# TheaQG/DiffusionModelsCustom

Hardware: NVIDIA B200
Metric: samples_per_s_T1000_ddpm_sampling (higher is better)
Workload: dtype fp16 operands, fp32 accumulate (fp32 state/update)

## Files before the change

### diffusionmodelscustom_b200/_native.py

```python
from __future__ import annotations

import ctypes as C
import os

_PKG = os.path.dirname(os.path.abspath(__file__))
LIB_PATH = os.environ.get("B2D_LIB") or os.path.join(_PKG, "libb200ddpm.so")

FAMILY_R, FAMILY_D = 0, 1
INTERP_MODES = {"bicubic": 0, "bilinear": 1, "nearest": 2}

SYMBOLS = ["b2d_last_error", "b2d_abi_version", "b2d_create", "b2d_destroy", "b2d_load_weights", "b2d_set_schedule",
           "b2d_set_conditioning", "b2d_forward", "b2d_sample", "b2d_sample_host", "b2d_last_launch_count", "b2d_debug_read", "b2d_profile_step",
           "b2d_op_conv2d", "b2d_op_layernorm", "b2d_op_attention", "b2d_op_attn_block", "b2d_op_attn_block_out", "b2d_op_instnorm", "b2d_op_posterior_update", "b2d_saturation_count", "b2d_debug_attn_trace", "b2d_ensemble_run",
           "b2d_op_noise_image", "b2d_op_weighted_mse", "b2d_op_eval_daily", "b2d_op_eval_pixel", "b2d_op_histogram", "b2d_encoder_forward", "b2d_decoder_forward", "b2d_op_final_layer",
           "b2d_set_timesteps", "b2d_op_ddim_update"]


class Config(C.Structure):
    _fields_ = [(n, C.c_int32) for n in ("family", "img_size", "max_batch", "c_hr", "c_out", "has_lsm", "has_topo",
                                         "cond_channels", "num_classes", "n_heads", "attn_ff", "debug_simt_conv",
                                         "interp_mode", "stem_embedding")]


class Tensor(C.Structure):
    _fields_ = [("name", C.c_char_p), ("data", C.c_void_p), ("ndim", C.c_int32), ("shape", C.c_int64 * 4)]


class OpProfile(C.Structure):
    _fields_ = [("name", C.c_char * 48), ("klass", C.c_char * 24), ("flops", C.c_double), ("bytes", C.c_double),
                ("ms", C.c_double)]


class NativeError(RuntimeError):
    pass


_lib = None


def lib():
    global _lib
    if _lib is None:
        if not os.path.exists(LIB_PATH):
            raise NativeError(f"{LIB_PATH} is missing: build it with `python -m diffusionmodelscustom_b200.build` "
                              "(there is no fallback path)")
        L = C.CDLL(LIB_PATH)
# ... 8 lines not shown
                                           C.c_void_p, C.c_int32, C.c_void_p]
        L.b2d_forward.argtypes = [C.c_void_p, C.c_void_p, C.c_void_p, C.c_void_p, C.c_int32, C.c_void_p]
        L.b2d_sample.argtypes = [C.c_void_p, C.c_void_p, C.c_void_p, C.c_uint64, C.c_uint64, C.c_float, C.c_int32,
                                 C.c_void_p]
        L.b2d_sample_host.argtypes = [C.c_void_p, C.c_void_p, C.c_void_p, C.c_void_p, C.c_void_p, C.c_int32, C.c_int32,
                                      C.c_void_p, C.c_void_p, C.c_uint64, C.c_uint64, C.c_float, C.c_int32]
        L.b2d_last_launch_count.argtypes = [C.c_void_p]
        L.b2d_last_launch_count.restype = C.c_int64
        L.b2d_debug_read.argtypes = [C.c_void_p, C.c_char_p, C.c_void_p, C.c_int64, C.POINTER(C.c_int32), C.POINTER(C.c_int32)]
        L.b2d_profile_step.argtypes = [C.c_void_p, C.c_void_p, C.c_void_p, C.c_int32, C.c_int32, C.POINTER(OpProfile),
                                       C.c_int32, C.POINTER(C.c_int32)]
        L.b2d_op_conv2d.argtypes = [C.c_void_p] * 5 + [C.c_int32, C.c_void_p] + [C.c_int32] * 12 + [C.c_void_p]
        L.b2d_op_layernorm.argtypes = [C.c_void_p] * 4 + [C.c_int32, C.c_int32, C.c_void_p]
        L.b2d_op_attention.argtypes = [C.c_void_p, C.c_void_p] + [C.c_int32] * 4 + [C.c_void_p]
        L.b2d_op_attn_block.argtypes = [C.c_void_p] * 5 + [C.c_int32] * 4 + [C.c_void_p]
        L.b2d_op_attn_block_out.argtypes = [C.c_void_p] * 7 + [C.c_int32] * 5 + [C.c_void_p]
        L.b2d_op_instnorm.argtypes = [C.c_void_p, C.c_void_p, C.c_void_p, C.c_int32, C.c_void_p, C.c_void_p] + \
                                     [C.c_int32] * 3 + [C.c_void_p]
        L.b2d_op_final_layer.argtypes = [C.c_void_p] * 4 + [C.c_int32] * 4 + [C.c_void_p]
        L.b2d_op_posterior_update.argtypes = [C.c_void_p] * 6 + [C.c_int32, C.c_int32, C.c_int64, C.c_uint64, C.c_uint64,
                                                                 C.c_float, C.c_void_p]
        L.b2d_set_timesteps.argtypes = [C.c_void_p, C.c_void_p, C.c_int32, C.c_float]
        L.b2d_op_ddim_update.argtypes = [C.c_void_p] * 4 + [C.c_int32] * 3 + [C.c_float, C.c_int32, C.c_int64, C.c_uint64,
                                                              C.c_uint64, C.c_float, C.c_void_p]
        L.b2d_op_noise_image.argtypes = [C.c_void_p] * 6 + [C.c_int32, C.c_int64, C.c_uint64, C.c_uint64, C.c_float, C.c_void_p]
        L.b2d_op_weighted_mse.argtypes = [C.c_void_p] * 3 + [C.c_float, C.c_float, C.c_void_p, C.c_int64, C.c_void_p]
        L.b2d_op_eval_daily.argtypes = [C.c_void_p] * 4 + [C.c_int32, C.c_int64, C.c_void_p]
        L.b2d_op_eval_pixel.argtypes = [C.c_void_p] * 5 + [C.c_int32, C.c_int64, C.c_void_p]
        L.b2d_op_histogram.argtypes = [C.c_void_p, C.c_int64, C.c_float, C.c_float, C.c_int32, C.c_void_p, C.c_void_p]
        L.b2d_encoder_forward.argtypes = [C.c_void_p, C.c_void_p, C.c_void_p, C.POINTER(C.c_void_p), C.c_int32, C.c_void_p]
        L.b2d_decoder_forward.argtypes = [C.c_void_p, C.POINTER(C.c_void_p), C.c_void_p, C.c_void_p, C.c_int32, C.c_void_p]
        L.b2d_saturation_count.argtypes = [C.c_int32]
        L.b2d_saturation_count.restype = C.c_uint32
        if L.b2d_abi_version() != 1:
            raise NativeError("libb200ddpm.so ABI version mismatch")
        _lib = L
    return _lib


def check(rc: int):
    if rc != 0:
        raise NativeError(f"b200ddpm error {rc}: {lib().b2d_last_error().decode(errors='replace')}")


def ptr(t):
    return None if t is None else t.data_ptr()
```

### diffusionmodelscustom_b200/csrc/attention_tc8.cuh

```cuda
#pragma once
#include "attention_tc6.cuh"

namespace b2d {

constexpr int AT8_THREADS = 160;
constexpr int AT8_EQ_BYTES = ATC_BLK * ATC_D * 2;
constexpr int AT8_EK_BYTES = (ATC_BN / 2) * ATC_D * 2;
constexpr int AT8_SMEM = 1024 + ATC_TILE_BYTES + ATC_KV_BYTES * 3 * ATC_STAGES + AT8_EQ_BYTES + AT8_EK_BYTES + 256;

constexpr float AT8_OFF_SFU = 7.0f, AT8_OFF_POLY = 22.0f;

__device__ __forceinline__ uint32_t ex2_pair_poly_off(float xa, float xb) {
    uint32_t h, xr, nf, f, p, r;
    asm("cvt.rn.relu.f16x2.f32 %0, %1, %2;" : "=r"(h) : "f"(xb), "f"(xa));
    asm("add.rn.f16x2 %0, %1, %2;" : "=r"(xr) : "r"(h), "r"(0x66006600u));
    asm("sub.rn.f16x2 %0, %1, %2;" : "=r"(nf) : "r"(xr), "r"(0x66006600u));
    asm("sub.rn.f16x2 %0, %1, %2;" : "=r"(f) : "r"(h), "r"(nf));
    asm("fma.rn.f16x2 %0, %1, %2, %3;" : "=r"(p) : "r"(0x2B0D2B0Du), "r"(f), "r"(0x33C333C3u));
    asm("fma.rn.f16x2 %0, %1, %2, %3;" : "=r"(p) : "r"(p), "r"(f), "r"(0x398C398Cu));
    asm("fma.rn.f16x2 %0, %1, %2, %3;" : "=r"(p) : "r"(p), "r"(f), "r"(0x3C003C00u));
    const uint32_t e = xr * 1024u - 0x01980000u;
    asm("mul.rn.f16x2 %0, %1, %2;" : "=r"(r) : "r"(p), "r"(e));
    return r;
}

template <int POLY>
__global__ void __launch_bounds__(AT8_THREADS, AT6_CTAS_PER_SM)
    attn_tc8_kernel(const __grid_constant__ CUtensorMap tm, const __grid_constant__ CUtensorMap tmkv, f16* __restrict__ o, int L,
                    int C, float scale_log2e) {
    pdl_launch_dependents();
    extern __shared__ uint8_t at8_raw[];
    uint8_t* smem = reinterpret_cast<uint8_t*>((reinterpret_cast<uintptr_t>(at8_raw) + 1023) & ~uintptr_t(1023));
    uint8_t* sQ = smem;
    uint8_t* sK = sQ + ATC_TILE_BYTES;
    uint8_t* sV = sK + ATC_STAGES * ATC_KV_BYTES;
    uint8_t* sEq = sV + ATC_STAGES * 2 * ATC_KV_BYTES;
    uint8_t* sEk = sEq + AT8_EQ_BYTES;
    uint64_t* bars = reinterpret_cast<uint64_t*>(sEk + AT8_EK_BYTES);
    constexpr int KV_FULL = 0, S_FULL = 4 , P_EMPTY = 6, Q_FULL = 7, NBARS = 8;
    uint32_t* tmem_slot = reinterpret_cast<uint32_t*>(bars + NBARS);
    const uint32_t bar0 = smem_u32(bars);

    const int warp = threadIdx.x >> 5, lane = threadIdx.x & 31;
    const int head = blockIdx.y, b = blockIdx.z;
    const int q0 = blockIdx.x * ATC_BLK;
    const int nb = L / ATC_BN;
    const int row_base = b * L;
    constexpr int IW = 4, NT = AT8_THREADS;

    if (warp == IW) {
        if (lane == 0) {
            tma_prefetch_desc(&tm);
            tma_prefetch_desc(&tmkv);
            for (int i = 0; i < NBARS; ++i) mbar_init(&bars[i], 1);
            fence_mbar_init();
        }
        __syncwarp();
        tmem_alloc(tmem_slot, AT3_TMEM_COLS);
        tmem_relinquish();
    }
    for (int i = threadIdx.x; i < ATC_STAGES * ATC_BN * 2; i += NT) {
        const int st = i / (ATC_BN * 2), r = i % (ATC_BN * 2);
// ... 44 lines not shown
        }
        __syncwarp();
        named_bar_sync(4, NT);
        if (elect_one()) {
            issue_s_half(0, 0);
            issue_s_half(0, 1);
        }
        __syncwarp();
        for (int j = 0; j < nb; ++j) {
#pragma unroll
            for (int ch = 0; ch < 2; ++ch) {
                named_bar_sync(1 + ch, NT);
                tc_fence_after();
                if (j + 1 < nb) {
                    if (elect_one()) issue_s_half(j + 1, ch);
                    __syncwarp();
                }
            }
            named_bar_sync(3, NT);
            tc_fence_after();
            if (elect_one()) {
                const uint64_t dv = dv0 + (uint64_t)((j & (ATC_STAGES - 1)) * (2 * ATC_KV_BYTES / 16));
#pragma unroll
                for (int kk = 0; kk < ATC_BN / 16; ++kk)
                    umma_f16_ts(tmem + AT3_O_COL, tmem + AT3_P_COL + kk * 8, dv + (uint64_t)(kk * (512 / 16)), idesc_o, (j | kk) != 0);
                umma_commit_a(bar0 + 8 * P_EMPTY);
                if (j >= 1 && j + 3 < nb) load_kv(j + 3);
            }
            __syncwarp();
        }
    } else {
        const uint32_t tl = tmem + ((uint32_t)(warp * 32) << 16);
        const int row = warp * 32 + lane;
        {
            mbar_wait_a(bar0 + 8 * Q_FULL, 0);
            const f162 sc = __float2half2_rn(scale_log2e);
            f162* qp = reinterpret_cast<f162*>(sQ + threadIdx.x * 32);
#pragma unroll
            for (int i = 0; i < 8; ++i) qp[i] = __hmul2(qp[i], sc);
            fence_proxy_async();
            named_bar_arrive(4, NT);
        }
        uint32_t* eq_row = reinterpret_cast<uint32_t*>(sEq + row * 32);
        float m_ref = 0.f;
        float m_eq = 0.f;
        float mb[2] = {0.f, 0.f};
        auto rescale_o = [&](float fac) {
            uint32_t ov[32];
            tmem_ld32(tl + AT3_O_COL, ov);
            tmem_ld_wait();
            uint32_t o0[16], o1[16];
#pragma unroll
            for (int i = 0; i < 16; ++i) {
                o0[i] = __float_as_uint(__uint_as_float(ov[i]) * fac);
                o1[i] = __float_as_uint(__uint_as_float(ov[16 + i]) * fac);
            }
            tmem_st16(tl + AT3_O_COL, o0);
            tmem_st16(tl + AT3_O_COL + 16, o1);
            tmem_st_wait();
        };
        auto rescale_p_first_half = [&](float fac) {
            tmem_st_wait();
            uint32_t pv[32];
            tmem_ld32(tl + AT3_P_COL, pv);
            tmem_ld_wait();
            uint32_t p0[16];
#pragma unroll
            for (int i = 0; i < 16; ++i) {
                const float2 f = unpack_h2(pv[i]);
                p0[i] = pack_h2_nosat(f.x * fac, f.y * fac);
            }
            tmem_st16(tl + AT3_P_COL, p0);
        };

        for (int j = 0; j < nb; ++j) {
            bool waited_p = false;
#pragma unroll
            for (int ch = 0; ch < 2; ++ch) {
                mbar_wait_a(bar0 + 8 * (S_FULL + ch), j & 1);
                tc_fence_after();
                uint32_t v[32];
                tmem_ld32(tl + ch * 32, v);
                tmem_ld_wait();
                tc_fence_before();
                named_bar_arrive(1 + ch, NT);
                const float d0 = m_ref - mb[ch];
                mb[ch] = m_eq;
                float mx[2] = {-INFINITY, -INFINITY};
#pragma unroll
                for (int i = 0; i < 32; i += 2) {
                    const int cls = (((i >> 1) & 7) < POLY) ? 1 : 0;
                    mx[cls] = fmaxf(mx[cls], fmaxf(__uint_as_float(v[i]), __uint_as_float(v[i + 1])));
                }
                const bool first = (j == 0) && (ch == 0);
                const bool slow = d0 != 0.0f || mx[0] > 8.0f + AT8_OFF_SFU || mx[1] > 8.0f + AT8_OFF_POLY || first;
                if (__any_sync(0xffffffffu, slow)) {
                    const float cm = fmaxf(mx[0] - AT8_OFF_SFU, mx[1] - AT8_OFF_POLY) - d0;
                    const bool move = cm > 8.0f || first;
                    float m_new = m_ref;
                    if (move) {
                        const float t = m_ref + cm;
                        const f16 hi = __float2half_rn(t);
                        const f16 lo = __float2half_rn(t - __half2float(hi));
                        m_new = __half2float(hi) + __half2float(lo);
                    }
                    if (__any_sync(0xffffffffu, move)) {
                        if (!waited_p) {
                            mbar_wait_a(bar0 + 8 * P_EMPTY, (j & 1) ^ 1);
                            tc_fence_after();
                            waited_p = true;
                        }
                        const float fac = move ? ex2_approx(m_ref - m_new) : 1.0f;
                        if (j > 0) rescale_o(fac);
                        if (ch == 1) rescale_p_first_half(fac);
                        if (j + 1 < nb) mbar_wait_a(bar0 + 8 * (S_FULL + 0), (j + 1) & 1);
                        if (ch == 0) mbar_wait_a(bar0 + 8 * (S_FULL + 1), j & 1);
                        else if (j + 1 < nb) mbar_wait_a(bar0 + 8 * (S_FULL + 1), (j + 1) & 1);
                        if (move) {
                            const f16 hi = __float2half_rn(m_new);
                            const f16 lo = __float2half_rn(m_new - __half2float(hi));
                            const uint32_t w = (uint32_t)__half_as_ushort(__hneg(hi)) | ((uint32_t)__half_as_ushort(__hneg(lo)) << 16);
                            eq_row[0] = w;
                            eq_row[4] = w;
                            m_eq = m_new;
                        }
                        fence_proxy_async();
                    }
                    const float shift = m_new - (m_ref - d0);
#pragma unroll
                    for (int i = 0; i < 32; ++i) v[i] = __float_as_uint(__uint_as_float(v[i]) - shift);
                    m_ref = m_new;
                }
                uint32_t pk[16];
#pragma unroll
                for (int idx = 0; idx < 16 + AT_PIPE; ++idx) {
                    if (idx < 16) {
                        const float s0 = __uint_as_float(v[2 * idx]), s1 = __uint_as_float(v[2 * idx + 1]);
                        if ((idx & 7) < POLY) {
                            pk[idx] = ex2_pair_poly_off(s0, s1);
                        } else {
                            v[2 * idx] = __float_as_uint(ex2_ordered(s0));
                            v[2 * idx + 1] = __float_as_uint(ex2_ordered(s1));
                        }
                    }
                    if (idx >= AT_PIPE) {
                        const int i = idx - AT_PIPE;
                        if ((i & 7) >= POLY) pk[i] = pack_h2_ordered(__uint_as_float(v[2 * i]), __uint_as_float(v[2 * i + 1]));
                    }
                }
                if (!waited_p) {
                    mbar_wait_a(bar0 + 8 * P_EMPTY, (j & 1) ^ 1);
                    tc_fence_after();
                    waited_p = true;
                }
                tmem_st16(tl + AT3_P_COL + ch * 16, pk);
            }
            tmem_st_wait();
            tc_fence_before();
            named_bar_arrive(3, NT);
        }
        mbar_wait_a(bar0 + 8 * P_EMPTY, (nb - 1) & 1);
        tc_fence_after();
        uint32_t ov[32];
        tmem_ld32(tl + AT3_O_COL, ov);
        tmem_ld_wait();
        const float inv = 1.0f / __uint_as_float(ov[16]);
        f16* op = o + ((size_t)(row_base + q0 + row)) * C + head * ATC_D;
        uint4 o0, o1;
        o0.x = pack_h2(__uint_as_float(ov[0]) * inv, __uint_as_float(ov[1]) * inv);
        o0.y = pack_h2(__uint_as_float(ov[2]) * inv, __uint_as_float(ov[3]) * inv);
        o0.z = pack_h2(__uint_as_float(ov[4]) * inv, __uint_as_float(ov[5]) * inv);
        o0.w = pack_h2(__uint_as_float(ov[6]) * inv, __uint_as_float(ov[7]) * inv);
        o1.x = pack_h2(__uint_as_float(ov[8]) * inv, __uint_as_float(ov[9]) * inv);
        o1.y = pack_h2(__uint_as_float(ov[10]) * inv, __uint_as_float(ov[11]) * inv);
        o1.z = pack_h2(__uint_as_float(ov[12]) * inv, __uint_as_float(ov[13]) * inv);
        o1.w = pack_h2(__uint_as_float(ov[14]) * inv, __uint_as_float(ov[15]) * inv);
        reinterpret_cast<uint4*>(op)[0] = o0;
        reinterpret_cast<uint4*>(op)[1] = o1;
    }
    tc_fence_before();
    __syncthreads();
    if (warp == IW) {
        tc_fence_after();
        tmem_dealloc(tmem, AT3_TMEM_COLS);
    }
}

inline int attn_tc8_poly() {
    static const int v = [] {
        const char* e = getenv("B2D_ATTN_POLY");
        const int p = e ? atoi(e) : 4;
        return p < 0 ? 0 : (p > 5 ? 5 : p);
    }();
    return v;
}

template <int POLY>
inline int attn_tc8_attr() {
    B2D_CUDA(cudaFuncSetAttribute(attn_tc8_kernel<POLY>, cudaFuncAttributeMaxDynamicSharedMemorySize, AT8_SMEM));
    B2D_CUDA(cudaFuncSetAttribute(attn_tc8_kernel<POLY>, cudaFuncAttributePreferredSharedMemoryCarveout, cudaSharedmemCarveoutMaxShared));
    return 0;
}
inline int attn_tc8_init_attrs() {
    B2D_TRY(attn_tc8_attr<0>());
    B2D_TRY(attn_tc8_attr<2>());
    B2D_TRY(attn_tc8_attr<3>());
    B2D_TRY(attn_tc8_attr<4>());
    B2D_TRY(attn_tc8_attr<5>());
    return 0;
}

inline int attn_tc8_launch(const AttnTcMaps& m, f16* o, int B, int L, int C, int heads, cudaStream_t st) {
    const float scale_log2e = 1.4426950408889634f / sqrtf((float)ATC_D);
    const dim3 grid(L / ATC_BLK, heads, B), block(AT8_THREADS);
    switch (attn_tc8_poly()) {
        case 0: case 1: B2D_CUDA(launch_k(attn_tc8_kernel<0>, grid, block, AT8_SMEM, st, m.q, m.kv, o, L, C, scale_log2e)); break;
        case 2: B2D_CUDA(launch_k(attn_tc8_kernel<2>, grid, block, AT8_SMEM, st, m.q, m.kv, o, L, C, scale_log2e)); break;
        case 3: B2D_CUDA(launch_k(attn_tc8_kernel<3>, grid, block, AT8_SMEM, st, m.q, m.kv, o, L, C, scale_log2e)); break;
        case 4: B2D_CUDA(launch_k(attn_tc8_kernel<4>, grid, block, AT8_SMEM, st, m.q, m.kv, o, L, C, scale_log2e)); break;
        default: B2D_CUDA(launch_k(attn_tc8_kernel<5>, grid, block, AT8_SMEM, st, m.q, m.kv, o, L, C, scale_log2e)); break;
    }
    return 0;
}

}
```

### diffusionmodelscustom_b200/csrc/b200ddpm.cu

```cuda
#include "../../include/b200ddpm.h"

#include <chrono>
#include <cmath>
#include <cstring>
#include <functional>
#include <map>
#include <memory>
#include <vector>

#include "attention.cuh"
#include "attention_tc.cuh"
#include "attention_tc2.cuh"
#include "attention_tc3.cuh"
#include "attention_tc3d32.cuh"
#include "attention_tc6.cuh"
#include "attention_tc8.cuh"
#include "attn_block.cuh"
#include "common.cuh"
#include "conv.cuh"
#include "conv_persist.cuh"
#include "elementwise.cuh"
#include "evalops.cuh"
#include "gemm_stream.cuh"
#include "norm_fused.cuh"
// ... 488 lines not shown
            auto pl = std::make_shared<AttnBlockPlan>();
            if (attn_block_plan_build(*pl, x, W<f16>(role + ".qkvln.w"), W<float>(role + ".qkvln.c1"), W<float>(role + ".qkvln.b"), ao,
                                      rows, C, L, heads) != 0) { err = -1; return; }
            static const bool no_out_fuse = getenv("B2D_NO_ATTN_OUT_FUSE") != nullptr;
            static const int out_fuse_maxc = getenv("B2D_ATTN_OUT_FUSE_MAXC") ? atoi(getenv("B2D_ATTN_OUT_FUSE_MAXC")) : 128;
            static const bool want_gather = getenv("B2D_ATTN_GATHER") != nullptr;
            const bool gather = !no_out_fuse && want_gather && attn_block_gather_supported(C, heads);
            fused_out = gather || (!no_out_fuse && attn_block_out_supported(C, heads) && C <= out_fuse_maxc);
            double fl = 6.0 * rows * C * C + 4.0 * (double)L * L * C * B, by = 4.0 * rows * C + 6.0 * C * C;
            if (fused_out) {
                float* ws = nullptr;
                if (!gather && h->alloc(&ws, attn_block_ws_floats(rows, C, heads)) != 0) { err = -2; return; }
                if (attn_block_plan_fuse_out(*pl, W<f16>(role + ".out.w"), W<float>(role + ".out.b"), x,
                                             h->cfg.attn_ff ? s_mid : out, ws, h->cfg.attn_ff ? 0 : final_act, gather ? 2 : 1) != 0) { err = -1; return; }
                fl += 2.0 * rows * C * C;
                by += 4.0 * rows * C + 2.0 * C * C;
            }
            ops.meta(role + ".attn", "attn_block", fl, by);
            ops.push_back([=](cudaStream_t st) { return attn_block_launch(*pl, st); });
        } else if (fold) {
            next_ln_c1 = W<float>(role + ".qkvln.c1");
            conv(x, hw, hw, C, qkv, 3 * C, 1, 1, 0, false, role + ".qkvln", nullptr, nullptr, 0, 0);
        } else {
            ops.meta(role + ".ln", "layernorm", 0, 4.0 * rows * C);
            ops.push_back([=](cudaStream_t st) { return layernorm_launch(x, g, b, xn, rows, C, st); });
            conv(xn, hw, hw, C, qkv, 3 * C, 1, 1, 0, false, role + ".qkv", nullptr, nullptr, 0, 0);
        }
        static const bool no_tc_attn = getenv("B2D_NO_TC_ATTN") != nullptr;
        if (fused_block) {
        } else if (attn_tc_supported(L, C, heads) && !no_tc_attn) {
            auto tmq = std::make_shared<AttnTcMaps>();
            if (attn_tc_make_map(tmq.get(), qkv, B, L, C) != 0) { err = -1; return; }
            ops.meta(role + ".sdpa", "attn_tc", 4.0 * (double)L * L * C * B, 8.0 * rows * C);
            static const int attn_v = getenv("B2D_ATTN_V") ? atoi(getenv("B2D_ATTN_V")) : 8;
            const int sms = h->num_sms;
            if (attn_v == 2 && attn_tc2_supported(L, C, heads))
                ops.push_back([=](cudaStream_t st) { return attn_tc2_launch(*tmq, ao, Bc, L, C, heads, sms, st); });
            else if (attn_v == 1)
                ops.push_back([=](cudaStream_t st) { return attn_tc_launch(*tmq, ao, Bc, L, C, heads, st); });
            else if (attn_v == 4) {
                auto tm4 = std::make_shared<AttnTcMaps>();
                if (attn_tc4_make_map(tm4.get(), qkv, B, L, C) != 0) { err = -1; return; }
                ops.push_back([=](cudaStream_t st) { return attn_tc4_launch(*tm4, ao, Bc, L, C, heads, st); });
            } else if (attn_v == 6)
                ops.push_back([=](cudaStream_t st) { return attn_tc6_launch<0>(*tmq, ao, Bc, L, C, heads, st); });
            else if (attn_v == 7)
                ops.push_back([=](cudaStream_t st) { return attn_tc6_launch<1>(*tmq, ao, Bc, L, C, heads, st); });
            else if (attn_v == 8)
                ops.push_back([=](cudaStream_t st) { return attn_tc8_launch(*tmq, ao, Bc, L, C, heads, st); });
            else
                ops.push_back([=](cudaStream_t st) { return attn_tc3_launch(*tmq, ao, Bc, L, C, heads, st); });
        } else if (attn_tc5_supported(L, C, heads) && !no_tc_attn) {
            auto tm5 = std::make_shared<AttnTcMaps>();
            if (attn_tc5_make_map(tm5.get(), qkv, B, L, C) != 0) { err = -1; return; }
            ops.meta(role + ".sdpa", "attn_tc32", 4.0 * (double)L * L * C * B, 8.0 * rows * C);
            ops.push_back([=](cudaStream_t st) { return attn_tc5_launch(*tm5, ao, Bc, L, C, heads, st); });
        } else {
            ops.meta(role + ".sdpa", "flash_attn", 4.0 * (double)L * L * C * B, 8.0 * rows * C);
            ops.push_back([=](cudaStream_t st) { return flash_attn_launch(qkv, ao, Bc, L, C, heads, st); });
        }
        if (!h->cfg.attn_ff) {
            if (!fused_out) conv(ao, hw, hw, C, out, C, 1, 1, 0, false, role + ".out", x, nullptr, 0, final_act);
        } else {
            f16* mid = s_mid;
            f16* h1 = s_h1;
            if (!fused_out) conv(ao, hw, hw, C, mid, C, 1, 1, 0, false, role + ".out", x, nullptr, 0, 0);
            const float* g2 = W<float>(role + ".ffln.g");
            const float* b2 = W<float>(role + ".ffln.b");
            if (fold) {
                next_ln_c1 = W<float>(role + ".ff1ln.c1");
                conv(mid, hw, hw, C, h1, C, 1, 1, 0, false, role + ".ff1ln", nullptr, nullptr, 0, 2);
            } else {
                ops.meta(role + ".ffln", "layernorm", 0, 4.0 * rows * C);
                ops.push_back([=](cudaStream_t st) { return layernorm_launch(mid, g2, b2, xn, rows, C, st); });
                conv(xn, hw, hw, C, h1, C, 1, 1, 0, false, role + ".ff1", nullptr, nullptr, 0, 2);
            }
            conv(h1, hw, hw, C, out, C, 1, 1, 0, false, role + ".ff2", mid, nullptr, 0, final_act);
        }
    }

    float* stats_slice(int C) {
// ... 925 lines not shown
        return gemm_stream_launch(gp, as_stream(stream));
    }
    B2D_TRY(conv_tc_init_attrs());
    B2D_TRY(conv_plan_build(pl, sms, impl != 4 && impl != 5));
    if (impl == 5) impl = 3;
    if (impl == 3 || (impl == 0 && conv_tcp_eligible(pl, sms))) {
        B2D_CHECK(pl.p.splits == 1, "shape not eligible for the persistent convolution (split-K plan)");
        B2D_TRY(conv_tcp_init_attrs());
        return conv_launch_tcp(pl, sms, as_stream(stream));
    }
    float* ws = nullptr;
    if (pl.ws_floats) {
        B2D_CUDA(cudaMalloc(&ws, pl.ws_floats * sizeof(float)));
        pl.p.ws = ws;
    }
    int rc = conv_launch_tc(pl, as_stream(stream));
    if (ws) {
        cudaStreamSynchronize(as_stream(stream));
        cudaFree(ws);
    }
    return rc;
}

int b2d_op_layernorm(const void* x, const float* gamma, const float* beta, void* y, int32_t rows, int32_t C, void* stream) {
    return layernorm_launch((const f16*)x, gamma, beta, (f16*)y, rows, C, as_stream(stream));
}

int b2d_op_attention(const void* qkv, void* o, int32_t B, int32_t L, int32_t C, int32_t heads, void* stream) {
    B2D_TRY(flash_attn_init_attrs());
    if (attn_tc_supported(L, C, heads) && getenv("B2D_NO_TC_ATTN") == nullptr) {
        B2D_TRY(attn_tc_init_attrs());
        AttnTcMaps tm;
        B2D_TRY(attn_tc_make_map(&tm, (const f16*)qkv, B, L, C));
        const int attn_v = getenv("B2D_ATTN_V") ? atoi(getenv("B2D_ATTN_V")) : 8;
        if (attn_v == 3) {
            B2D_TRY(attn_tc3_init_attrs());
            return attn_tc3_launch(tm, (f16*)o, B, L, C, heads, as_stream(stream));
        }
        if (attn_v == 8) {
            B2D_TRY(attn_tc8_init_attrs());
            return attn_tc8_launch(tm, (f16*)o, B, L, C, heads, as_stream(stream));
        }
        if (attn_v == 6 || attn_v == 7) {
            B2D_TRY(attn_tc6_init_attrs());
            return attn_v == 6 ? attn_tc6_launch<0>(tm, (f16*)o, B, L, C, heads, as_stream(stream))
                               : attn_tc6_launch<1>(tm, (f16*)o, B, L, C, heads, as_stream(stream));
        }
        if (attn_v == 4) {
            B2D_TRY(attn_tc3_init_attrs());
            B2D_TRY(attn_tc4_make_map(&tm, (const f16*)qkv, B, L, C));
            return attn_tc4_launch(tm, (f16*)o, B, L, C, heads, as_stream(stream));
        }
        if (attn_v == 2 && attn_tc2_supported(L, C, heads)) {
            B2D_TRY(attn_tc2_init_attrs());
            int dev = 0, sms = 148;
            cudaGetDevice(&dev);
            cudaDeviceGetAttribute(&sms, cudaDevAttrMultiProcessorCount, dev);
            return attn_tc2_launch(tm, (f16*)o, B, L, C, heads, sms, as_stream(stream));
        }
        return attn_tc_launch(tm, (f16*)o, B, L, C, heads, as_stream(stream));
    }
    if (attn_tc5_supported(L, C, heads) && getenv("B2D_NO_TC_ATTN") == nullptr) {
        B2D_TRY(attn_tc5_init_attrs());
        AttnTcMaps tm5;
        B2D_TRY(attn_tc5_make_map(&tm5, (const f16*)qkv, B, L, C));
        return attn_tc5_launch(tm5, (f16*)o, B, L, C, heads, as_stream(stream));
    }
// ... 184 lines not shown
                      void* stream) {
    B2D_CHECK(gen && eval && mae_out && rmse_out && n_samples >= 1 && hw >= 1, "bad argument");
    eval_daily_kernel<<<n_samples, 256, 0, as_stream(stream)>>>(gen, eval, mae_out, rmse_out, (size_t)hw);
    B2D_CUDA(cudaGetLastError());
    return 0;
}

int b2d_op_eval_pixel(const float* gen, const float* eval, float* mae_out, float* rmse_out, float* bias_out, int32_t n_samples,
                      int64_t hw, void* stream) {
    B2D_CHECK(gen && eval && mae_out && rmse_out && bias_out && n_samples >= 1 && hw >= 1, "bad argument");
    eval_pixel_kernel<<<(unsigned)((hw + 255) / 256), 256, 0, as_stream(stream)>>>(gen, eval, mae_out, rmse_out, bias_out, n_samples, (size_t)hw);
    B2D_CUDA(cudaGetLastError());
    return 0;
}

int b2d_op_histogram(const float* x, int64_t n, float lo, float hi, int32_t bins, unsigned long long* counts_dev, void* stream) {
    B2D_CHECK(x && counts_dev && n >= 0 && bins >= 1 && bins <= HIST_MAX_BINS && hi > lo, "bad argument");
    cudaStream_t st = as_stream(stream);
    B2D_CUDA(cudaMemsetAsync(counts_dev, 0, (size_t)bins * 8, st));
    if (n == 0) return 0;
    const int blocks = (int)std::min<int64_t>((n + 255) / 256, 148 * 4);
    histogram_kernel<<<blocks, 256, (size_t)bins * 4, st>>>(x, (size_t)n, lo, hi, bins, counts_dev);
    B2D_CUDA(cudaGetLastError());
    return 0;
}

int b2d_debug_attn_trace(long long* out_host, int32_t max_elems) {
    B2D_CHECK(out_host && max_elems >= AT2_TRACE_BLOCKS * 12, "trace buffer too small");
    B2D_CUDA(cudaDeviceSynchronize());
    B2D_CUDA(cudaMemcpyFromSymbol(out_host, g_at2_trace, sizeof(long long) * AT2_TRACE_BLOCKS * 12));
    return AT2_TRACE_BLOCKS;
}

unsigned int b2d_saturation_count(int32_t reset) {
    unsigned int v = 0;
    if (cudaMemcpyFromSymbol(&v, g_sat_count, sizeof(v)) != cudaSuccess) return 0xFFFFFFFFu;
    if (reset) {
        const unsigned int z = 0;
        cudaMemcpyToSymbol(g_sat_count, &z, sizeof(z));
    }
    return v;
}

}
```

### include/b200ddpm.h

```cpp
#ifndef B200DDPM_H
#define B200DDPM_H

#include <stddef.h>
#include <stdint.h>

#ifdef __cplusplus
extern "C" {
#endif

#define B2D_ABI_VERSION 1

typedef struct b2d_handle b2d_handle;

enum { B2D_FAMILY_R = 0,
       B2D_FAMILY_D = 1   };

typedef struct b2d_config {
    int32_t family;
    int32_t img_size;
    int32_t max_batch;
    int32_t c_hr;
    int32_t c_out;
    int32_t has_lsm;
    int32_t has_topo;
// ... 38 lines not shown
int b2d_set_timesteps(b2d_handle* h, const int32_t* timesteps_host, int32_t n, float eta);
int b2d_op_ddim_update(float* x, const float* eps, const float* z_or_null, const float* alpha_hat, int32_t T, int32_t t,
                       int32_t t_prev, float eta, int32_t B, int64_t per_sample, uint64_t seed, uint64_t sample_offset,
                       float noise_scale, void* stream);

int b2d_sample_host(b2d_handle* h, float* x_inout_host, const float* lsm_host, const float* topo_host,
                    const float* cond_host, int32_t cond_h, int32_t cond_w, const int64_t* y_host,
                    const float* noise_host, uint64_t seed, uint64_t sample_offset, float noise_scale, int32_t B);

typedef struct b2d_ensemble_job {
    int32_t n_dates, members, sub_batch;
    int32_t first, count;
    const float* lsm;
    const float* topo;
    const float* cond;
    int32_t cond_h, cond_w;
    const int64_t* y;
    float* out;
    uint64_t seed;
    float noise_scale;
    float xT_scale;
} b2d_ensemble_job;
typedef struct b2d_ensemble_stats {
    int32_t sub_batches;
    int32_t out_pinned;
    int64_t launches;
    double gather_ms;
    double wall_ms;
} b2d_ensemble_stats;
int b2d_ensemble_run(b2d_handle* h, const b2d_ensemble_job* job, b2d_ensemble_stats* stats);

unsigned int b2d_saturation_count(int32_t reset);

int64_t b2d_last_launch_count(const b2d_handle* h);
typedef struct b2d_op_profile {
    char name[48];
    char klass[24];
    double flops;
    double bytes;
    double ms;
} b2d_op_profile;
int b2d_profile_step(b2d_handle* h, const float* x, const int64_t* t_host, int32_t B, int32_t reps, b2d_op_profile* out,
                     int32_t max_ops, int32_t* n_ops);

int b2d_debug_read(b2d_handle* h, const char* name, float* out_host, int64_t max_elems, int32_t* C_out, int32_t* hw_out);

int b2d_op_noise_image(const float* x0, const int64_t* t_dev, const float* alpha_hat, const float* noise_or_null, float* x_t,
                       float* noise_out, int32_t B, int64_t per_sample, uint64_t seed, uint64_t sample_offset, float noise_scale,
                       void* stream);
int b2d_op_weighted_mse(const float* input, const float* target, const float* sdf_or_null, float max_land_weight,
                        float min_sea_weight, float* out_scalar_dev, int64_t n, void* stream);
int b2d_op_eval_daily(const float* gen, const float* eval, float* mae_out, float* rmse_out, int32_t n_samples, int64_t hw,
                      void* stream);
int b2d_op_eval_pixel(const float* gen, const float* eval, float* mae_out, float* rmse_out, float* bias_out, int32_t n_samples,
                      int64_t hw, void* stream);
int b2d_op_histogram(const float* x, int64_t n, float lo, float hi, int32_t bins, unsigned long long* counts_dev, void* stream);

int b2d_debug_attn_trace(long long* out_host, int32_t max_elems);

int b2d_op_conv2d(const void* in_f16, const void* w_packed_f16, const float* bias, const void* residual_f16,
                  const float* post_add, int32_t post_stride, void* out_f16, int32_t B, int32_t Hi, int32_t Wi,
                  int32_t Cin, int32_t Cout, int32_t R, int32_t S, int32_t stride, int32_t pad, int32_t convt,
                  int32_t act, int32_t impl, void* stream);
int b2d_op_layernorm(const void* x_f16, const float* gamma, const float* beta, void* y_f16, int32_t rows, int32_t C,
                     void* stream);
int b2d_op_attention(const void* qkv_f16, void* o_f16, int32_t B, int32_t L, int32_t C, int32_t heads, void* stream);
// ... 18 lines not shown
```

Before: 25.82.

## Skip per-tile softmax max scan using Cauchy-Schwarz bound from key-norm table

Adds a pre-pass kernel that computes, for every 32-key tile and head, an upper bound on the key norms. The attention kernel computes each query's norm and uses the product as a bound on the scores, so the per-chunk row-max reduction and rescale logic run only when that bound could exceed the current reference. This removes max-scan work from the softmax warps, at the cost of an extra launch, an allocation and a table read per chunk. It is enabled by default (variant 9) only when L is at least 4096, and optional atomic counters can record how often the slow path runs.

After: 26.43, median of 6. 1.02x the previous value.

```diff
diff --git a/diffusionmodelscustom_b200/_native.py b/diffusionmodelscustom_b200/_native.py
--- a/diffusionmodelscustom_b200/_native.py
+++ b/diffusionmodelscustom_b200/_native.py
@@ -11,7 +11,7 @@
 
 SYMBOLS = ["b2d_last_error", "b2d_abi_version", "b2d_create", "b2d_destroy", "b2d_load_weights", "b2d_set_schedule",
            "b2d_set_conditioning", "b2d_forward", "b2d_sample", "b2d_sample_host", "b2d_last_launch_count", "b2d_debug_read", "b2d_profile_step",
-           "b2d_op_conv2d", "b2d_op_layernorm", "b2d_op_attention", "b2d_op_attn_block", "b2d_op_attn_block_out", "b2d_op_instnorm", "b2d_op_posterior_update", "b2d_saturation_count", "b2d_debug_attn_trace", "b2d_ensemble_run",
+           "b2d_op_conv2d", "b2d_op_layernorm", "b2d_op_attention", "b2d_op_attn_block", "b2d_op_attn_block_out", "b2d_op_instnorm", "b2d_op_posterior_update", "b2d_saturation_count", "b2d_op_attn_kmax", "b2d_attn_scan_stats", "b2d_debug_attn_trace", "b2d_ensemble_run",
            "b2d_op_noise_image", "b2d_op_weighted_mse", "b2d_op_eval_daily", "b2d_op_eval_pixel", "b2d_op_histogram", "b2d_encoder_forward", "b2d_decoder_forward", "b2d_op_final_layer",
            "b2d_set_timesteps", "b2d_op_ddim_update"]
 
@@ -86,6 +86,8 @@
         L.b2d_decoder_forward.argtypes = [C.c_void_p, C.POINTER(C.c_void_p), C.c_void_p, C.c_void_p, C.c_int32, C.c_void_p]
         L.b2d_saturation_count.argtypes = [C.c_int32]
         L.b2d_saturation_count.restype = C.c_uint32
+        L.b2d_op_attn_kmax.argtypes = [C.c_void_p, C.c_void_p] + [C.c_int32] * 3 + [C.c_void_p]
+        L.b2d_attn_scan_stats.argtypes = [C.c_int32, C.POINTER(C.c_uint64)]
         if L.b2d_abi_version() != 1:
             raise NativeError("libb200ddpm.so ABI version mismatch")
         _lib = L
diff --git a/diffusionmodelscustom_b200/csrc/attention_tc8.cuh b/diffusionmodelscustom_b200/csrc/attention_tc8.cuh
--- a/diffusionmodelscustom_b200/csrc/attention_tc8.cuh
+++ b/diffusionmodelscustom_b200/csrc/attention_tc8.cuh
@@ -24,10 +24,14 @@
     return r;
 }
 
-template <int POLY>
+__device__ unsigned long long g_attn_scan[4];
+
+__device__ __forceinline__ float at8_bound_limit(float m_ref) { return m_ref + 8.0f - 0x1p-8f - fabsf(m_ref) * 0x1p-10f; }
+
+template <int POLY, bool BOUND>
 __global__ void __launch_bounds__(AT8_THREADS, AT6_CTAS_PER_SM)
     attn_tc8_kernel(const __grid_constant__ CUtensorMap tm, const __grid_constant__ CUtensorMap tmkv, f16* __restrict__ o, int L,
-                    int C, float scale_log2e) {
+                    int C, float scale_log2e, const float* __restrict__ kmax, unsigned long long* __restrict__ stats) {
     pdl_launch_dependents();
     extern __shared__ uint8_t at8_raw[];
     uint8_t* smem = reinterpret_cast<uint8_t*>((reinterpret_cast<uintptr_t>(at8_raw) + 1023) & ~uintptr_t(1023));
@@ -138,12 +142,22 @@
     } else {
         const uint32_t tl = tmem + ((uint32_t)(warp * 32) << 16);
         const int row = warp * 32 + lane;
+        float qn_up = 0.f;
         {
             mbar_wait_a(bar0 + 8 * Q_FULL, 0);
             const f162 sc = __float2half2_rn(scale_log2e);
             f162* qp = reinterpret_cast<f162*>(sQ + threadIdx.x * 32);
-#pragma unroll
-            for (int i = 0; i < 8; ++i) qp[i] = __hmul2(qp[i], sc);
+            float qq = 0.f;
+#pragma unroll
+            for (int i = 0; i < 8; ++i) {
+                const f162 sq = __hmul2(qp[i], sc);
+                qp[i] = sq;
+                if constexpr (BOUND) {
+                    const float2 f = __half22float2(sq);
+                    qq = fmaf(f.x, f.x, fmaf(f.y, f.y, qq));
+                }
+            }
+            qn_up = sqrtf(qq) * (1.0f + 0x1p-10f);
             fence_proxy_async();
             named_bar_arrive(4, NT);
         }
@@ -151,6 +165,8 @@
         float m_ref = 0.f;
         float m_eq = 0.f;
         float mb[2] = {0.f, 0.f};
+        float lim = at8_bound_limit(m_ref);
+        const float* kt = kmax + ((size_t)b * gridDim.y + head) * (L / 32);
         auto rescale_o = [&](float fac) {
             uint32_t ov[32];
             tmem_ld32(tl + AT3_O_COL, ov);
@@ -183,6 +199,8 @@
             bool waited_p = false;
 #pragma unroll
             for (int ch = 0; ch < 2; ++ch) {
+                float km = 0.f;
+                if constexpr (BOUND) km = __ldg(kt + 2 * j + ch);
                 mbar_wait_a(bar0 + 8 * (S_FULL + ch), j & 1);
                 tc_fence_after();
                 uint32_t v[32];
@@ -192,50 +210,68 @@
                 named_bar_arrive(1 + ch, NT);
                 const float d0 = m_ref - mb[ch];
                 mb[ch] = m_eq;
-                float mx[2] = {-INFINITY, -INFINITY};
-#pragma unroll
-                for (int i = 0; i < 32; i += 2) {
-                    const int cls = (((i >> 1) & 7) < POLY) ? 1 : 0;
-                    mx[cls] = fmaxf(mx[cls], fmaxf(__uint_as_float(v[i]), __uint_as_float(v[i + 1])));
-                }
                 const bool first = (j == 0) && (ch == 0);
-                const bool slow = d0 != 0.0f || mx[0] > 8.0f + AT8_OFF_SFU || mx[1] > 8.0f + AT8_OFF_POLY || first;
-                if (__any_sync(0xffffffffu, slow)) {
-                    const float cm = fmaxf(mx[0] - AT8_OFF_SFU, mx[1] - AT8_OFF_POLY) - d0;
-                    const bool move = cm > 8.0f || first;
-                    float m_new = m_ref;
-                    if (move) {
-                        const float t = m_ref + cm;
-                        const f16 hi = __float2half_rn(t);
-                        const f16 lo = __float2half_rn(t - __half2float(hi));
-                        m_new = __half2float(hi) + __half2float(lo);
+                bool over = false, need = true;
+                if constexpr (BOUND) {
+                    over = !(qn_up * km <= lim);
+                    need = first || d0 != 0.0f || over;
+                }
+                if (!BOUND || __any_sync(0xffffffffu, need)) {
+                    if (BOUND && stats != nullptr) {
+                        const unsigned ob = __ballot_sync(0xffffffffu, over);
+                        if (lane == 0) {
+                            atomicAdd(&stats[1], 1ull);
+                            if (ob) {
+                                atomicAdd(&stats[2], 1ull);
+                                atomicAdd(&stats[3], (unsigned long long)__popc(ob));
+                            }
+                        }
                     }
-                    if (__any_sync(0xffffffffu, move)) {
-                        if (!waited_p) {
-                            mbar_wait_a(bar0 + 8 * P_EMPTY, (j & 1) ^ 1);
-                            tc_fence_after();
-                            waited_p = true;
+                    float mx[2] = {-INFINITY, -INFINITY};
+#pragma unroll
+                    for (int i = 0; i < 32; i += 2) {
+                        const int cls = (((i >> 1) & 7) < POLY) ? 1 : 0;
+                        mx[cls] = fmaxf(mx[cls], fmaxf(__uint_as_float(v[i]), __uint_as_float(v[i + 1])));
+                    }
+                    const bool slow = d0 != 0.0f || mx[0] > 8.0f + AT8_OFF_SFU || mx[1] > 8.0f + AT8_OFF_POLY || first;
+                    if (__any_sync(0xffffffffu, slow)) {
+                        const float cm = fmaxf(mx[0] - AT8_OFF_SFU, mx[1] - AT8_OFF_POLY) - d0;
+                        const bool move = cm > 8.0f || first;
+                        float m_new = m_ref;
+                        if (move) {
+                            const float t = m_ref + cm;
+                            const f16 hi = __float2half_rn(t);
+                            const f16 lo = __float2half_rn(t - __half2float(hi));
+                            m_new = __half2float(hi) + __half2float(lo);
                         }
-                        const float fac = move ? ex2_approx(m_ref - m_new) : 1.0f;
-                        if (j > 0) rescale_o(fac);
-                        if (ch == 1) rescale_p_first_half(fac);
-                        if (j + 1 < nb) mbar_wait_a(bar0 + 8 * (S_FULL + 0), (j + 1) & 1);
-                        if (ch == 0) mbar_wait_a(bar0 + 8 * (S_FULL + 1), j & 1);
-                        else if (j + 1 < nb) mbar_wait_a(bar0 + 8 * (S_FULL + 1), (j + 1) & 1);
-                        if (move) {
-                            const f16 hi = __float2half_rn(m_new);
-                            const f16 lo = __float2half_rn(m_new - __half2float(hi));
-                            const uint32_t w = (uint32_t)__half_as_ushort(__hneg(hi)) | ((uint32_t)__half_as_ushort(__hneg(lo)) << 16);
-                            eq_row[0] = w;
-                            eq_row[4] = w;
-                            m_eq = m_new;
+                        if (__any_sync(0xffffffffu, move)) {
+                            if (!waited_p) {
+                                mbar_wait_a(bar0 + 8 * P_EMPTY, (j & 1) ^ 1);
+                                tc_fence_after();
+                                waited_p = true;
+                            }
+                            const float fac = move ? ex2_approx(m_ref - m_new) : 1.0f;
+                            if (j > 0) rescale_o(fac);
+                            if (ch == 1) rescale_p_first_half(fac);
+                            if (j + 1 < nb) mbar_wait_a(bar0 + 8 * (S_FULL + 0), (j + 1) & 1);
+                            if (ch == 0) mbar_wait_a(bar0 + 8 * (S_FULL + 1), j & 1);
+                            else if (j + 1 < nb) mbar_wait_a(bar0 + 8 * (S_FULL + 1), (j + 1) & 1);
+                            if (move) {
+                                const f16 hi = __float2half_rn(m_new);
+                                const f16 lo = __float2half_rn(m_new - __half2float(hi));
+                                const uint32_t w = (uint32_t)__half_as_ushort(__hneg(hi)) | ((uint32_t)__half_as_ushort(__hneg(lo)) << 16);
+                                eq_row[0] = w;
+                                eq_row[4] = w;
+                                m_eq = m_new;
+                            }
+                            fence_proxy_async();
                         }
-                        fence_proxy_async();
+                        const float shift = m_new - (m_ref - d0);
+#pragma unroll
+                        for (int i = 0; i < 32; ++i) v[i] = __float_as_uint(__uint_as_float(v[i]) - shift);
+                        m_ref = m_new;
+                        if constexpr (BOUND) lim = at8_bound_limit(m_ref);
                     }
-                    const float shift = m_new - (m_ref - d0);
-#pragma unroll
-                    for (int i = 0; i < 32; ++i) v[i] = __float_as_uint(__uint_as_float(v[i]) - shift);
-                    m_ref = m_new;
                 }
                 uint32_t pk[16];
 #pragma unroll
@@ -283,6 +319,7 @@
         o1.w = pack_h2(__uint_as_float(ov[14]) * inv, __uint_as_float(ov[15]) * inv);
         reinterpret_cast<uint4*>(op)[0] = o0;
         reinterpret_cast<uint4*>(op)[1] = o1;
+        if (BOUND && stats != nullptr && lane == 0) atomicAdd(&stats[0], 2ull * nb);
     }
     tc_fence_before();
     __syncthreads();
@@ -301,32 +338,92 @@
     return v;
 }
 
-template <int POLY>
+__global__ void __launch_bounds__(1024) attn_kmax_kernel(const f16* __restrict__ qkv, float* __restrict__ kmax, int L, int C) {
+    pdl_launch_dependents();
+    __shared__ unsigned s_max[32];
+    const int heads = C / ATC_D, h0 = blockIdx.y * 32;
+    const int hn = heads - h0 < 32 ? heads - h0 : 32;
+    const int r = threadIdx.x / hn, hd = threadIdx.x - r * hn;
+    const size_t key = (size_t)blockIdx.x * 32 + r;
+    if (threadIdx.x < hn) s_max[threadIdx.x] = 0u;
+    pdl_wait();
+    const uint4* kp = reinterpret_cast<const uint4*>(qkv + key * 3 * C + C + (h0 + hd) * ATC_D);
+    const uint4 a = __ldg(kp), c = __ldg(kp + 1);
+    const uint32_t w[8] = {a.x, a.y, a.z, a.w, c.x, c.y, c.z, c.w};
+    float s = 0.f;
+#pragma unroll
+    for (int i = 0; i < 8; ++i) {
+        const float2 f = unpack_h2(w[i]);
+        s = fmaf(f.x, f.x, fmaf(f.y, f.y, s));
+    }
+    float n = sqrtf(s) * (1.0f + 0x1p-10f);
+    if (!(n <= INFINITY)) n = INFINITY;
+    __syncthreads();
+    atomicMax(&s_max[hd], __float_as_uint(n));
+    __syncthreads();
+    if (threadIdx.x < hn) {
+        const int b = (int)((size_t)blockIdx.x * 32 / L), t = (int)((size_t)blockIdx.x % (L / 32));
+        kmax[((size_t)b * heads + h0 + threadIdx.x) * (L / 32) + t] = __uint_as_float(s_max[threadIdx.x]);
+    }
+}
+
+inline bool attn_tc8_bound_pays(int L) { return L >= 4096; }
+
+inline size_t attn_kmax_floats(int B, int L, int C) { return (size_t)B * (C / ATC_D) * (L / 32); }
+
+inline int attn_kmax_launch(const f16* qkv, float* kmax, int B, int L, int C, cudaStream_t st) {
+    B2D_CHECK(C > 0 && C % ATC_D == 0 && L > 0 && L % 32 == 0, "shape not eligible for the key-norm table");
+    const int heads = C / ATC_D;
+    B2D_CUDA(launch_k(attn_kmax_kernel, dim3(B * (L / 32), (heads + 31) / 32), dim3(32 * (heads < 32 ? heads : 32)), 0, st, qkv, kmax, L, C));
+    return 0;
+}
+
+inline bool& attn_scan_stats_on() {
+    static bool on = false;
+    return on;
+}
+inline unsigned long long* attn_scan_stats_ptr() {
+    if (!attn_scan_stats_on()) return nullptr;
+    void* p = nullptr;
+    return cudaGetSymbolAddress(&p, g_attn_scan) == cudaSuccess ? static_cast<unsigned long long*>(p) : nullptr;
+}
+
+template <int POLY, bool BOUND>
 inline int attn_tc8_attr() {
-    B2D_CUDA(cudaFuncSetAttribute(attn_tc8_kernel<POLY>, cudaFuncAttributeMaxDynamicSharedMemorySize, AT8_SMEM));
-    B2D_CUDA(cudaFuncSetAttribute(attn_tc8_kernel<POLY>, cudaFuncAttributePreferredSharedMemoryCarveout, cudaSharedmemCarveoutMaxShared));
+    B2D_CUDA(cudaFuncSetAttribute(attn_tc8_kernel<POLY, BOUND>, cudaFuncAttributeMaxDynamicSharedMemorySize, AT8_SMEM));
+    B2D_CUDA(cudaFuncSetAttribute(attn_tc8_kernel<POLY, BOUND>, cudaFuncAttributePreferredSharedMemoryCarveout, cudaSharedmemCarveoutMaxShared));
     return 0;
 }
+template <bool BOUND>
+inline int attn_tc8_attrs() {
+    B2D_TRY((attn_tc8_attr<0, BOUND>()));
+    B2D_TRY((attn_tc8_attr<2, BOUND>()));
+    B2D_TRY((attn_tc8_attr<3, BOUND>()));
+    B2D_TRY((attn_tc8_attr<4, BOUND>()));
+    B2D_TRY((attn_tc8_attr<5, BOUND>()));
+    return 0;
+}
 inline int attn_tc8_init_attrs() {
-    B2D_TRY(attn_tc8_attr<0>());
-    B2D_TRY(attn_tc8_attr<2>());
-    B2D_TRY(attn_tc8_attr<3>());
-    B2D_TRY(attn_tc8_attr<4>());
-    B2D_TRY(attn_tc8_attr<5>());
-    return 0;
-}
-
-inline int attn_tc8_launch(const AttnTcMaps& m, f16* o, int B, int L, int C, int heads, cudaStream_t st) {
+    B2D_TRY(attn_tc8_attrs<false>());
+    return attn_tc8_attrs<true>();
+}
+
+template <bool BOUND>
+inline int attn_tc8_launch_t(const AttnTcMaps& m, f16* o, int B, int L, int C, int heads, const float* kmax, cudaStream_t st) {
     const float scale_log2e = 1.4426950408889634f / sqrtf((float)ATC_D);
     const dim3 grid(L / ATC_BLK, heads, B), block(AT8_THREADS);
+    unsigned long long* stats = BOUND ? attn_scan_stats_ptr() : nullptr;
     switch (attn_tc8_poly()) {
-        case 0: case 1: B2D_CUDA(launch_k(attn_tc8_kernel<0>, grid, block, AT8_SMEM, st, m.q, m.kv, o, L, C, scale_log2e)); break;
-        case 2: B2D_CUDA(launch_k(attn_tc8_kernel<2>, grid, block, AT8_SMEM, st, m.q, m.kv, o, L, C, scale_log2e)); break;
-        case 3: B2D_CUDA(launch_k(attn_tc8_kernel<3>, grid, block, AT8_SMEM, st, m.q, m.kv, o, L, C, scale_log2e)); break;
-        case 4: B2D_CUDA(launch_k(attn_tc8_kernel<4>, grid, block, AT8_SMEM, st, m.q, m.kv, o, L, C, scale_log2e)); break;
-        default: B2D_CUDA(launch_k(attn_tc8_kernel<5>, grid, block, AT8_SMEM, st, m.q, m.kv, o, L, C, scale_log2e)); break;
+        case 0: case 1: B2D_CUDA(launch_k(attn_tc8_kernel<0, BOUND>, grid, block, AT8_SMEM, st, m.q, m.kv, o, L, C, scale_log2e, kmax, stats)); break;
+        case 2: B2D_CUDA(launch_k(attn_tc8_kernel<2, BOUND>, grid, block, AT8_SMEM, st, m.q, m.kv, o, L, C, scale_log2e, kmax, stats)); break;
+        case 3: B2D_CUDA(launch_k(attn_tc8_kernel<3, BOUND>, grid, block, AT8_SMEM, st, m.q, m.kv, o, L, C, scale_log2e, kmax, stats)); break;
+        case 4: B2D_CUDA(launch_k(attn_tc8_kernel<4, BOUND>, grid, block, AT8_SMEM, st, m.q, m.kv, o, L, C, scale_log2e, kmax, stats)); break;
+        default: B2D_CUDA(launch_k(attn_tc8_kernel<5, BOUND>, grid, block, AT8_SMEM, st, m.q, m.kv, o, L, C, scale_log2e, kmax, stats)); break;
     }
     return 0;
 }
-
-}
+inline int attn_tc8_launch(const AttnTcMaps& m, f16* o, int B, int L, int C, int heads, cudaStream_t st, const float* kmax = nullptr) {
+    return kmax ? attn_tc8_launch_t<true>(m, o, B, L, C, heads, kmax, st) : attn_tc8_launch_t<false>(m, o, B, L, C, heads, nullptr, st);
+}
+
+}
diff --git a/diffusionmodelscustom_b200/csrc/b200ddpm.cu b/diffusionmodelscustom_b200/csrc/b200ddpm.cu
--- a/diffusionmodelscustom_b200/csrc/b200ddpm.cu
+++ b/diffusionmodelscustom_b200/csrc/b200ddpm.cu
@@ -544,9 +544,17 @@
             auto tmq = std::make_shared<AttnTcMaps>();
             if (attn_tc_make_map(tmq.get(), qkv, B, L, C) != 0) { err = -1; return; }
             ops.meta(role + ".sdpa", "attn_tc", 4.0 * (double)L * L * C * B, 8.0 * rows * C);
-            static const int attn_v = getenv("B2D_ATTN_V") ? atoi(getenv("B2D_ATTN_V")) : 8;
+            static const int attn_v = getenv("B2D_ATTN_V") ? atoi(getenv("B2D_ATTN_V")) : 9;
             const int sms = h->num_sms;
-            if (attn_v == 2 && attn_tc2_supported(L, C, heads))
+            if (attn_v == 9 && attn_tc8_bound_pays(L)) {
+                float* kmax = nullptr;
+                if (h->alloc(&kmax, attn_kmax_floats(B, L, C)) != 0) { err = -2; return; }
+                const Op sdpa = ops.pending;
+                ops.meta(role + ".kmax", "attn_kmax", 0, 2.0 * rows * C + 4.0 * attn_kmax_floats(B, L, C));
+                ops.push_back([=](cudaStream_t st) { return attn_kmax_launch(qkv, kmax, Bc, L, C, st); });
+                ops.pending = sdpa;
+                ops.push_back([=](cudaStream_t st) { return attn_tc8_launch(*tmq, ao, Bc, L, C, heads, st, kmax); });
+            } else if (attn_v == 2 && attn_tc2_supported(L, C, heads))
                 ops.push_back([=](cudaStream_t st) { return attn_tc2_launch(*tmq, ao, Bc, L, C, heads, sms, st); });
             else if (attn_v == 1)
                 ops.push_back([=](cudaStream_t st) { return attn_tc_launch(*tmq, ao, Bc, L, C, heads, st); });
@@ -558,7 +566,7 @@
                 ops.push_back([=](cudaStream_t st) { return attn_tc6_launch<0>(*tmq, ao, Bc, L, C, heads, st); });
             else if (attn_v == 7)
                 ops.push_back([=](cudaStream_t st) { return attn_tc6_launch<1>(*tmq, ao, Bc, L, C, heads, st); });
-            else if (attn_v == 8)
+            else if (attn_v == 8 || attn_v == 9)
                 ops.push_back([=](cudaStream_t st) { return attn_tc8_launch(*tmq, ao, Bc, L, C, heads, st); });
             else
                 ops.push_back([=](cudaStream_t st) { return attn_tc3_launch(*tmq, ao, Bc, L, C, heads, st); });
@@ -1550,7 +1558,16 @@
         B2D_TRY(attn_tc_init_attrs());
         AttnTcMaps tm;
         B2D_TRY(attn_tc_make_map(&tm, (const f16*)qkv, B, L, C));
-        const int attn_v = getenv("B2D_ATTN_V") ? atoi(getenv("B2D_ATTN_V")) : 8;
+        const int attn_v = getenv("B2D_ATTN_V") ? atoi(getenv("B2D_ATTN_V")) : 9;
+        if (attn_v == 9) {
+            B2D_TRY(attn_tc8_init_attrs());
+            float* kmax = nullptr;
+            B2D_CUDA(cudaMallocAsync(&kmax, attn_kmax_floats(B, L, C) * sizeof(float), as_stream(stream)));
+            int rc = attn_kmax_launch((const f16*)qkv, kmax, B, L, C, as_stream(stream));
+            if (rc == 0) rc = attn_tc8_launch(tm, (f16*)o, B, L, C, heads, as_stream(stream), kmax);
+            cudaFreeAsync(kmax, as_stream(stream));
+            return rc;
+        }
         if (attn_v == 3) {
             B2D_TRY(attn_tc3_init_attrs());
             return attn_tc3_launch(tm, (f16*)o, B, L, C, heads, as_stream(stream));
@@ -1801,6 +1818,22 @@
     return AT2_TRACE_BLOCKS;
 }
 
+int b2d_op_attn_kmax(const void* qkv, float* kmax, int32_t B, int32_t L, int32_t C, void* stream) {
+    return attn_kmax_launch((const f16*)qkv, kmax, B, L, C, as_stream(stream));
+}
+
+int b2d_attn_scan_stats(int32_t enable, uint64_t* out) {
+    unsigned long long v[4] = {0, 0, 0, 0};
+    B2D_CUDA(cudaDeviceSynchronize());
+    B2D_CUDA(cudaMemcpyFromSymbol(v, g_attn_scan, sizeof(v)));
+    if (out)
+        for (int i = 0; i < 4; ++i) out[i] = v[i];
+    const unsigned long long z[4] = {0, 0, 0, 0};
+    B2D_CUDA(cudaMemcpyToSymbol(g_attn_scan, z, sizeof(z)));
+    attn_scan_stats_on() = enable != 0;
+    return 0;
+}
+
 unsigned int b2d_saturation_count(int32_t reset) {
     unsigned int v = 0;
     if (cudaMemcpyFromSymbol(&v, g_sat_count, sizeof(v)) != cudaSuccess) return 0xFFFFFFFFu;
diff --git a/include/b200ddpm.h b/include/b200ddpm.h
--- a/include/b200ddpm.h
+++ b/include/b200ddpm.h
@@ -94,6 +94,9 @@
 
 unsigned int b2d_saturation_count(int32_t reset);
 
+int b2d_op_attn_kmax(const void* qkv, float* kmax, int32_t B, int32_t L, int32_t C, void* stream);
+int b2d_attn_scan_stats(int32_t enable, uint64_t* out);
+
 int64_t b2d_last_launch_count(const b2d_handle* h);
 typedef struct b2d_op_profile {
     char name[48];
```
